# fchchen/omni-recall-rag

Measured on AMD Instinct MI355X. Metric: queries/sec at top-k=10 over N x 3072-d chunks; score delta vs C# reference in `parity`, higher is better.
Workload: dtype i8 screen + f32*f32->f64 exact re-score; 1 GPU; C3: 10000000 chunks x 3072-d fp32 on one GPU, batch=256 queries per step, top-k=10, full hybrid (cosine+keyword+recency), candidate_limit=corpus; corpus_rows=10000000

## Files before the change

include/omnirecall_hip.h:

```cpp
#ifndef OMNIRECALL_HIP_H
#define OMNIRECALL_HIP_H

#include <stddef.h>
#include <stdint.h>

#ifdef __cplusplus
extern "C" {
#endif

#define ORR_ABI_VERSION 1

typedef enum orr_status {
    ORR_OK      = 0,
    ORR_EINVAL  = -1,
    ORR_ENOMEM  = -2,
    ORR_EDEVICE = -3,
    ORR_ECOMM   = -4,
    ORR_EDIM    = -5,
    ORR_ESTATE  = -6,
    ORR_ELIMIT  = -7
} orr_status;

typedef struct orr_index orr_index;

// ... 233 lines not shown
int orr_index_get_rows(orr_index *idx, int64_t n, const int64_t *row_ids , int32_t dim,
                       float *out_emb , uint8_t *out_found );

int orr_search_shard_in_scope(orr_index *idx, int32_t B, int32_t dim, const float *q,
                              const uint8_t *terms_utf8, const uint32_t *term_off, const uint32_t *query_term_off,
                              int64_t now_ticks, int32_t kprime, int64_t candidate_limit, int32_t topk, int32_t pass,
                              const orr_scope *scope, int64_t scope_before, orr_candidate *out);

int orr_search_shard_in_scopes(orr_index *idx, int32_t B, int32_t dim, const float *q,
                               const uint8_t *terms_utf8, const uint32_t *term_off, const uint32_t *query_term_off,
                               int64_t now_ticks, int32_t kprime, int64_t candidate_limit, int32_t topk, int32_t pass,
                               int32_t n_scopes, const orr_scope *const *scopes, const int32_t *query_scope ,
                               const int64_t *scope_before , orr_candidate *out);

int orr_index_set_option(orr_index *idx, const char *name, int64_t value);

int orr_index_screen_dots(orr_index *idx, int32_t B, int32_t dim, const float *q, float *out);

int orr_index_screen_i8_dots(orr_index *idx, int32_t B, int32_t dim, const float *q, int32_t form, int32_t nt_rows,
                             int32_t *out_dots, int8_t *out_iq, int8_t *out_ie);

int orr_index_screen_i8_consts(orr_index *idx, int32_t B, int32_t dim, const float *q, float *out_scale, float *out_rel_err,
                               float *out_rel_hat, float *out_rowf, float *out_s1, double *out_err2, double *out_err2_level1,
                               int8_t *out_iq2);

int orr_index_screen_i8_stream_dots(orr_index *idx, int32_t B, int32_t dim, const float *q, int32_t unit16, int32_t *out_dots);

int orr_index_pass_dots(orr_index *idx, int32_t kernel, int32_t B, int32_t dim, const float *q, float *out);

typedef struct orr_screen_capture {
    int32_t B;
    int32_t kth;
    uint32_t cap;
    int32_t screen;
    int32_t tile_form;
    int32_t scope;
    int32_t floor_form;
    int32_t reserved;
    int64_t n;
    int64_t prefix_rows;
    double eps3;
    double eps1;
} orr_screen_capture;
int orr_index_capture_screen(orr_index *idx, int32_t enabled);
int orr_index_captured_screen(orr_index *idx, orr_screen_capture *info, int32_t B, uint32_t cap, uint64_t *out_floor_key, double *out_L,
                              uint32_t *out_cnt, uint64_t *out_key, uint32_t *out_pos);

int orr_index_pair_dots(orr_index *idx, int32_t n_lists, const uint32_t *list_off ,
                        const int64_t *positions , int32_t stride ,
                        double *out );

int orr_index_keyword_bitmaps(orr_index *idx, int32_t n_terms, const uint8_t *terms_utf8, const uint32_t *term_off, int32_t form,
                              int32_t mid, int64_t out_words_per_term, uint32_t *out_bitmaps, uint8_t *out_alias, int64_t *out_info);

int orr_index_set_profiling(orr_index *idx, int32_t enabled);
int orr_index_kernel_stats(orr_index *idx, orr_kernel_stat *out, int32_t cap);

int orr_index_search_stats(orr_index *idx, orr_search_stats *out, int32_t reset);

typedef struct orr_cluster orr_cluster;
int        orr_cluster_create(const int32_t *devices, int32_t n_shards, int32_t dim, int64_t capacity_rows_per_shard,
                              orr_cluster **out);
void       orr_cluster_destroy(orr_cluster *c);
int32_t    orr_cluster_shards(const orr_cluster *c);
orr_index *orr_cluster_shard(orr_cluster *c, int32_t i);
int        orr_cluster_seal(orr_cluster *c);
int64_t    orr_cluster_rows(const orr_cluster *c);
int        orr_cluster_search_batch(orr_cluster *c, int32_t B, int32_t dim, const float *q_host,
                                    const uint8_t *terms_utf8, const uint32_t *term_off,
                                    const uint32_t *query_term_off, int64_t now_ticks, int32_t topk,
                                    int64_t candidate_limit, int64_t *out_rows, double *out_scores,
                                    int32_t *out_counts);
int        orr_cluster_search_batch_scoped(orr_cluster *c, int32_t B, int32_t dim, const float *q_host,
                                           const uint8_t *terms_utf8, const uint32_t *term_off,
                                           const uint32_t *query_term_off, int64_t now_ticks, int32_t topk,
                                           int64_t candidate_limit, int64_t n_scope_ids, const int64_t *scope_ids,
                                           const uint64_t *scope_off, int64_t *out_rows, double *out_scores,
                                           int32_t *out_counts);
int        orr_cluster_search_batch_masked(orr_cluster *c, int32_t B, int32_t dim, const float *q_host,
                                           const uint8_t *terms_utf8, const uint32_t *term_off,
                                           const uint32_t *query_term_off, int64_t now_ticks, int32_t topk,
                                           int64_t candidate_limit, int64_t n_scope_ids, const int64_t *scope_ids,
                                           int64_t *out_rows, double *out_scores, int32_t *out_counts);
int        orr_cluster_search_stats(orr_cluster *c, orr_search_stats *out, int32_t reset);
int        orr_cluster_set_option(orr_cluster *c, const char *name, int64_t value);
int        orr_cluster_compact(orr_cluster *c, int64_t *out_removed);

int        orr_cluster_insert_rows(orr_cluster *c, int32_t shard, int64_t n, int32_t dim, const float *emb,
                                   const int64_t *created_ticks, const uint8_t *content_lower,
                                   const uint64_t *content_off, const int64_t *row_ids, int64_t *out_inserted);

typedef struct orr_cluster_scope orr_cluster_scope;
int     orr_cluster_scope_create(orr_cluster *c, int64_t n_ids, const int64_t *ids , orr_cluster_scope **out);
int     orr_cluster_scope_create_ticks(orr_cluster *c, int64_t ticks_from, int64_t ticks_to, orr_cluster_scope **out);
int     orr_cluster_scope_create_terms(orr_cluster *c, int32_t n_terms, const uint8_t *terms_utf8 , const uint32_t *term_off ,
                                       int32_t mode, orr_cluster_scope **out);
int     orr_cluster_scope_create_near(orr_cluster *c, int32_t n_probes, int32_t dim, const float *probes ,
                                      double min_cosine, int32_t mode, orr_cluster_scope **out);
int     orr_cluster_scope_add_ids(orr_cluster_scope *s, int64_t n_ids, const int64_t *ids , int64_t *out_added);
int     orr_cluster_scope_combine(orr_cluster_scope *dst, int32_t op, const orr_cluster_scope *src);
int64_t orr_cluster_scope_rows(const orr_cluster_scope *s);
int     orr_cluster_scope_row_ids(orr_cluster_scope *s, int64_t cap, int64_t *out_ids , int64_t *out_n);
const orr_scope *orr_cluster_scope_shard(const orr_cluster_scope *s, int32_t i);
void    orr_cluster_scope_destroy(orr_cluster_scope *s);

int orr_cluster_search_batch_in_scope(orr_cluster *c, int32_t B, int32_t dim, const float *q_host,
// ... 59 lines not shown
```

omni-recall-rag_amd/_native.py:

```python
from __future__ import annotations

import ctypes as C
import os

_PKG = os.path.dirname(os.path.abspath(__file__))
HIP_LIB_PATH = os.environ.get("ORR_HIP_LIB") or os.path.join(_PKG, "libomnirecall_hip.so")
HOST_LIB_PATH = os.path.join(_PKG, "libomnirecall_host.so")


class OrrError(RuntimeError):
    def __init__(self, code: int, message: str):
        super().__init__(f"libomnirecall_hip status {code}: {message}")
        self.code = code


ORR_OK, ORR_EINVAL, ORR_ENOMEM, ORR_EDEVICE, ORR_ECOMM, ORR_EDIM, ORR_ESTATE = 0, -1, -2, -3, -4, -5, -6
ORR_ELIMIT = -7
ORR_CAND_TRAILER, ORR_CAND_DOT_EXACT, ORR_CAND_DEAD = 1, 2, 16
ORR_SCOPE_AND, ORR_SCOPE_OR, ORR_SCOPE_ANDNOT = 0, 1, 2
ORR_TERMS_ALL, ORR_TERMS_ANY = 0, 1
ORR_NEAR_ALL, ORR_NEAR_ANY = 0, 1
ORR_KEY_NONE = -(1 << 63)


# ... 122 lines not shown
hip.orr_keys_centroid_index.argtypes = [_vp, _vp, C.POINTER(_vp), _vp, _vp]
hip.orr_index_get_rows.restype = C.c_int
hip.orr_index_get_rows.argtypes = [_vp, _i64, _vp, _i32, _vp, _vp]
hip.orr_search_shard_in_scope.restype = C.c_int
hip.orr_search_shard_in_scope.argtypes = [_vp, _i32, _i32, _vp, _vp, _vp, _vp, _i64, _i32, _i64, _i32, _i32, _vp, _i64, _vp]
hip.orr_search_shard_in_scopes.restype = C.c_int
hip.orr_search_shard_in_scopes.argtypes = [_vp, _i32, _i32, _vp, _vp, _vp, _vp, _i64, _i32, _i64, _i32, _i32, _i32, _vp, _vp, _vp, _vp]
hip.orr_search_shard_ex.restype = C.c_int
hip.orr_search_shard_ex.argtypes = [_vp, _i32, _i32, _vp, _vp, _vp, _vp, _i64, _i32, _i64, _i32, _i32, _vp]
hip.orr_merge_candidates_ex.restype = C.c_int
hip.orr_merge_candidates_ex.argtypes = [_i32, _i32, _i32, _vp, _i32, _i32, _vp, _vp, _i64, _i32, _vp, _vp, _vp, _vp, _vp]
hip.orr_merge_candidates.restype = C.c_int
hip.orr_merge_candidates.argtypes = [_i32, _i32, _i32, _vp, _i32, _i32, _vp, _vp, _i64, _i32, _vp, _vp, _vp, _vp]
hip.orr_index_save.restype = C.c_int
hip.orr_index_save.argtypes = [_vp, C.c_char_p]
hip.orr_index_load.restype = C.c_int
hip.orr_index_load.argtypes = [C.POINTER(OrrConfig), C.c_char_p, C.POINTER(_vp)]
hip.orr_index_set_option.restype = C.c_int
hip.orr_index_set_option.argtypes = [_vp, C.c_char_p, _i64]
hip.orr_index_delete_rows.restype = C.c_int
hip.orr_index_delete_rows.argtypes = [_vp, _i64, _vp, _vp]
hip.orr_index_update_rows.restype = C.c_int
hip.orr_index_update_rows.argtypes = [_vp, _i64, _vp, _i32, _vp, _vp]
hip.orr_index_insert_rows.restype = C.c_int
hip.orr_index_insert_rows.argtypes = [_vp, _i64, _i32, _vp, _vp, _vp, _vp, _vp, _vp]
hip.orr_cluster_insert_rows.restype = C.c_int
hip.orr_cluster_insert_rows.argtypes = [_vp, _i32, _i64, _i32, _vp, _vp, _vp, _vp, _vp, _vp]
hip.orr_index_compact.restype = C.c_int
hip.orr_index_compact.argtypes = [_vp, _vp]
hip.orr_cluster_compact.restype = C.c_int
hip.orr_cluster_compact.argtypes = [_vp, _vp]
hip.orr_index_live_rows.restype = _i64
hip.orr_index_live_rows.argtypes = [_vp]
hip.orr_index_view.restype = C.c_int
hip.orr_index_view.argtypes = [_vp, C.POINTER(_vp)]
hip.orr_index_screen_dots.restype = C.c_int
hip.orr_index_screen_dots.argtypes = [_vp, _i32, _i32, _vp, _vp]
hip.orr_index_screen_i8_dots.restype = C.c_int
hip.orr_index_screen_i8_dots.argtypes = [_vp, _i32, _i32, _vp, _i32, _i32, _vp, _vp, _vp]
hip.orr_index_screen_i8_consts.restype = C.c_int
hip.orr_index_screen_i8_consts.argtypes = [_vp, _i32, _i32, _vp, _vp, _vp, _vp, _vp, _vp, _vp, _vp, _vp]
hip.orr_index_screen_i8_stream_dots.restype = C.c_int
hip.orr_index_screen_i8_stream_dots.argtypes = [_vp, _i32, _i32, _vp, _i32, _vp]
hip.orr_index_pass_dots.restype = C.c_int
hip.orr_index_pass_dots.argtypes = [_vp, _i32, _i32, _i32, _vp, _vp]
hip.orr_index_capture_screen.restype = C.c_int
hip.orr_index_capture_screen.argtypes = [_vp, _i32]
hip.orr_index_captured_screen.restype = C.c_int
hip.orr_index_captured_screen.argtypes = [_vp, C.POINTER(OrrScreenCapture), _i32, C.c_uint32, _vp, _vp, _vp, _vp, _vp]
hip.orr_index_pair_dots.restype = C.c_int
hip.orr_index_pair_dots.argtypes = [_vp, _i32, _vp, _vp, _i32, _vp]
hip.orr_index_keyword_bitmaps.restype = C.c_int
hip.orr_index_keyword_bitmaps.argtypes = [_vp, _i32, _vp, _vp, _i32, _i32, _i64, _vp, _vp, _vp]
hip.orr_index_set_profiling.restype = C.c_int
hip.orr_index_set_profiling.argtypes = [_vp, _i32]
hip.orr_index_kernel_stats.restype = C.c_int
hip.orr_index_kernel_stats.argtypes = [_vp, _vp, _i32]
hip.orr_index_search_stats.restype = C.c_int
hip.orr_index_search_stats.argtypes = [_vp, C.POINTER(OrrSearchStats), _i32]
hip.orr_cluster_create.restype = C.c_int
hip.orr_cluster_create.argtypes = [_vp, _i32, _i32, _i64, C.POINTER(_vp)]
hip.orr_cluster_destroy.restype = None
hip.orr_cluster_destroy.argtypes = [_vp]
hip.orr_cluster_shards.restype = _i32
hip.orr_cluster_shards.argtypes = [_vp]
hip.orr_cluster_shard.restype = _vp
hip.orr_cluster_shard.argtypes = [_vp, _i32]
hip.orr_cluster_seal.restype = C.c_int
hip.orr_cluster_seal.argtypes = [_vp]
hip.orr_cluster_rows.restype = _i64
hip.orr_cluster_rows.argtypes = [_vp]
hip.orr_cluster_search_batch.restype = C.c_int
hip.orr_cluster_search_batch.argtypes = [_vp, _i32, _i32, _vp, _vp, _vp, _vp, _i64, _i32, _i64, _vp, _vp, _vp]
hip.orr_cluster_search_batch_scoped.restype = C.c_int
hip.orr_cluster_search_batch_scoped.argtypes = [_vp, _i32, _i32, _vp, _vp, _vp, _vp, _i64, _i32, _i64, _i64, _vp, _vp, _vp, _vp, _vp]
hip.orr_cluster_search_batch_masked.restype = C.c_int
hip.orr_cluster_search_batch_masked.argtypes = [_vp, _i32, _i32, _vp, _vp, _vp, _vp, _i64, _i32, _i64, _i64, _vp, _vp, _vp, _vp]
hip.orr_cluster_set_option.restype = C.c_int
hip.orr_cluster_set_option.argtypes = [_vp, C.c_char_p, _i64]
hip.orr_cluster_search_stats.restype = C.c_int
hip.orr_cluster_search_stats.argtypes = [_vp, C.POINTER(OrrSearchStats), _i32]
hip.orr_cluster_scope_create.restype = C.c_int
hip.orr_cluster_scope_create.argtypes = [_vp, _i64, _vp, C.POINTER(_vp)]
hip.orr_cluster_scope_create_ticks.restype = C.c_int
hip.orr_cluster_scope_create_ticks.argtypes = [_vp, _i64, _i64, C.POINTER(_vp)]
hip.orr_cluster_scope_create_terms.restype = C.c_int
hip.orr_cluster_scope_create_terms.argtypes = [_vp, _i32, _vp, _vp, _i32, C.POINTER(_vp)]
hip.orr_cluster_scope_create_near.restype = C.c_int
hip.orr_cluster_scope_create_near.argtypes = [_vp, _i32, _i32, _vp, C.c_double, _i32, C.POINTER(_vp)]
hip.orr_cluster_scope_add_ids.restype = C.c_int
hip.orr_cluster_scope_add_ids.argtypes = [_vp, _i64, _vp, _vp]
hip.orr_cluster_scope_combine.restype = C.c_int
hip.orr_cluster_scope_combine.argtypes = [_vp, _i32, _vp]
hip.orr_cluster_scope_rows.restype = _i64
hip.orr_cluster_scope_rows.argtypes = [_vp]
hip.orr_cluster_scope_row_ids.restype = C.c_int
hip.orr_cluster_scope_row_ids.argtypes = [_vp, _i64, _vp, _vp]
hip.orr_cluster_scope_shard.restype = _vp
hip.orr_cluster_scope_shard.argtypes = [_vp, _i32]
hip.orr_cluster_scope_destroy.restype = None
hip.orr_cluster_scope_destroy.argtypes = [_vp]
hip.orr_cluster_search_batch_in_scope.restype = C.c_int
hip.orr_cluster_search_batch_in_scope.argtypes = [_vp, _i32, _i32, _vp, _vp, _vp, _vp, _i64, _i32, _i64, _vp, _vp, _vp, _vp]
hip.orr_cluster_search_batch_in_scopes.restype = C.c_int
hip.orr_cluster_search_batch_in_scopes.argtypes = [_vp, _i32, _i32, _vp, _vp, _vp, _vp, _i64, _i32, _i64, _i32, _vp, _vp, _vp, _vp, _vp]
hip.orr_cluster_search_range_cosine.restype = C.c_int
# ... 55 lines not shown
host.orrh_store_import_cosmos_json.restype = C.c_int
host.orrh_store_import_cosmos_json.argtypes = [_vp, C.c_char_p, _i64, _vp, _vp]
host.orrh_store_export_cosmos_json.restype = C.c_int
host.orrh_store_export_cosmos_json.argtypes = [_vp, C.POINTER(_vp), C.POINTER(_i64)]
host.orrh_store_chunk_count.restype = _i64
host.orrh_store_chunk_count.argtypes = [_vp]
host.orrh_service_create.restype = _vp
host.orrh_service_create.argtypes = [_vp, _i32, _i64]
host.orrh_service_stats.restype = None
host.orrh_service_stats.argtypes = [_vp, _vp, _vp, _vp]
host.orrh_service_tombstoned_rows.restype = _i64
host.orrh_service_tombstoned_rows.argtypes = [_vp]
host.orrh_service_compactions.restype = _i64
host.orrh_service_compactions.argtypes = [_vp]
host.orrh_service_delta_merges.restype = _i64
host.orrh_service_delta_merges.argtypes = [_vp]
host.orrh_service_updated_rows.restype = _i64
host.orrh_service_updated_rows.argtypes = [_vp]
host.orrh_service_inserted_rows.restype = _i64
host.orrh_service_inserted_rows.argtypes = [_vp]
host.orrh_service_set_option.restype = C.c_int
host.orrh_service_set_option.argtypes = [_vp, C.c_char_p, _i64]
host.orrh_service_destroy.restype = None
host.orrh_service_destroy.argtypes = [_vp]
host.orrh_service_search_json.restype = C.c_int
host.orrh_service_search_json.argtypes = [_vp, C.c_char_p, _vp, _i32, _i32, _i64, C.POINTER(_vp), C.POINTER(_i64)]
host.orrh_service_search_documents_json.restype = C.c_int
host.orrh_service_search_documents_json.argtypes = [_vp, C.c_char_p, _vp, _i32, _i32, _i64, C.POINTER(C.c_char_p), _i32, C.POINTER(_vp), C.POINTER(_i64)]
host.orrh_free.restype = None
host.orrh_free.argtypes = [_vp]
host.orrh_batcher_create.restype = _vp
host.orrh_batcher_create.argtypes = [_vp, _i32, _i32]
host.orrh_batcher_destroy.restype = None
host.orrh_batcher_destroy.argtypes = [_vp]
host.orrh_batcher_search.restype = C.c_int
host.orrh_batcher_search.argtypes = [_vp, _i32, _vp, _vp, _vp, _i32, _i64, _i32, _i64, _vp, _vp, _vp]
host.orrh_batcher_search_at.restype = C.c_int
host.orrh_batcher_search_at.argtypes = [_vp, _i32, _vp, _vp, _vp, _i32, _i64, _i32, _i64, _vp, _vp, _vp, _vp]
host.orrh_batcher_stats.restype = None
host.orrh_batcher_stats.argtypes = [_vp, _vp, _vp, _vp]
host.orrh_batcher_create.restype = _vp
host.orrh_batcher_create.argtypes = [_vp, _i32, _i32]
host.orrh_batcher_destroy.restype = None
host.orrh_batcher_destroy.argtypes = [_vp]
host.orrh_batcher_search.restype = C.c_int
host.orrh_batcher_search.argtypes = [_vp, _i32, _vp, _vp, _vp, _i32, _i64, _i32, _i64, _vp, _vp, _vp]
host.orrh_batcher_stats.restype = None
host.orrh_batcher_stats.argtypes = [_vp, _vp, _vp, _vp]

EXPORTED_HIP_SYMBOLS = [
    "orr_abi_version", "orr_device_count", "orr_last_error", "orr_index_create", "orr_index_destroy",
    "orr_index_append", "orr_index_seal", "orr_index_rows", "orr_index_dim", "orr_search_batch",
    "orr_search_shard", "orr_search_shard_ex", "orr_search_batch_scoped", "orr_search_batch_masked", "orr_search_batch_masked_groups", "orr_search_shard_scoped", "orr_search_shard_masked", "orr_index_scope_count", "orr_merge_candidates", "orr_merge_candidates_ex", "orr_index_set_profiling", "orr_index_kernel_stats",
    "orr_index_save", "orr_index_load", "orr_index_set_row_base", "orr_index_set_option", "orr_index_screen_dots", "orr_index_screen_i8_dots", "orr_index_screen_i8_consts", "orr_index_screen_i8_stream_dots", "orr_index_pass_dots", "orr_index_capture_screen", "orr_index_captured_screen", "orr_index_keyword_bitmaps", "orr_index_view",
    "orr_index_delete_rows", "orr_index_update_rows", "orr_index_insert_rows", "orr_cluster_insert_rows", "orr_index_live_rows", "orr_index_compact", "orr_cluster_compact", "orr_index_search_stats",
    "orr_cluster_create", "orr_cluster_destroy", "orr_cluster_shards", "orr_cluster_shard", "orr_cluster_seal", "orr_cluster_rows",
    "orr_cluster_search_batch", "orr_cluster_search_batch_scoped", "orr_cluster_search_batch_masked", "orr_cluster_search_stats", "orr_cluster_set_option",
    "orr_scope_create", "orr_scope_create_ticks", "orr_scope_create_terms", "orr_scope_create_near", "orr_scope_add_ids", "orr_scope_combine", "orr_scope_rows", "orr_scope_row_ids", "orr_scope_destroy",
    "orr_search_batch_in_scope", "orr_search_batch_in_scopes", "orr_search_shard_in_scope", "orr_search_shard_in_scopes", "orr_search_range_cosine", "orr_search_range_cosine_bulk",
    "orr_search_batch_diverse", "orr_index_pair_dots",
    "orr_keys_create", "orr_keys_set", "orr_keys_get", "orr_keys_rows", "orr_keys_destroy", "orr_scope_create_keys", "orr_search_batch_per_key",
    "orr_keys_groups", "orr_keys_centroids", "orr_scope_centroid",
    "orr_keys_centroid_index", "orr_index_get_rows",
    "orr_cluster_scope_create", "orr_cluster_scope_create_ticks", "orr_cluster_scope_create_terms", "orr_cluster_scope_create_near", "orr_cluster_scope_add_ids", "orr_cluster_scope_combine",
    "orr_cluster_scope_rows", "orr_cluster_scope_row_ids", "orr_cluster_scope_shard", "orr_cluster_scope_destroy", "orr_cluster_search_batch_in_scope",
    "orr_cluster_search_batch_in_scopes", "orr_cluster_search_range_cosine", "orr_cluster_search_range_cosine_bulk",
    "orr_cluster_search_batch_diverse", "orr_cluster_pair_dots",
    "orr_cluster_keys_create", "orr_cluster_keys_set", "orr_cluster_keys_get", "orr_cluster_keys_rows", "orr_cluster_keys_shard", "orr_cluster_keys_destroy",
    "orr_cluster_scope_create_keys", "orr_cluster_search_batch_per_key",
    "orr_cluster_keys_groups", "orr_cluster_keys_centroids", "orr_cluster_scope_centroid",
]
EXPORTED_HOST_SYMBOLS = ["orrh_is_blank", "orrh_lower_invariant", "orrh_query_terms", "orrh_build_snippet",
                         "orrh_round4", "orrh_has_sufficient_evidence", "orrh_format_score_f4", "orrh_last_error", "orrh_store_create", "orrh_store_destroy",
                         "orrh_store_upsert_document", "orrh_store_upsert_chunks", "orrh_store_delete_document",
                         "orrh_store_chunk_count", "orrh_store_import_cosmos_json", "orrh_store_export_cosmos_json", "orrh_service_create", "orrh_service_destroy",
                         "orrh_service_search_json", "orrh_service_search_documents_json", "orrh_service_stats", "orrh_service_tombstoned_rows", "orrh_service_compactions", "orrh_service_delta_merges", "orrh_service_updated_rows", "orrh_service_inserted_rows", "orrh_service_set_option", "orrh_free", "orrh_batcher_create", "orrh_batcher_destroy",
                         "orrh_batcher_search", "orrh_batcher_search_at", "orrh_batcher_stats"]


def check(status: int) -> None:
    if status != ORR_OK:
        raise OrrError(status, (hip.orr_last_error() or b"").decode("utf-8", "replace"))
```

omni-recall-rag_amd/csrc/orr_api.hip:

```cpp
#include <hip/hip_runtime.h>

#include <algorithm>
#include <cmath>
#include <cstdarg>
#include <cstdio>
#include <chrono>
#include <pthread.h>
#include <dlfcn.h>
#include <atomic>
#include <condition_variable>
#include <functional>
#include <cstring>
#include <limits>
#include <mutex>
#include <shared_mutex>
#include <deque>
#include <new>
#include <numeric>
#include <string>
#include <string_view>
#include <thread>
#include <unordered_map>
#include <vector>

// ... 5382 lines not shown
            HIP_TRY(orr::launch_scope_terms_bases(kws.view.term_word_off, n_distinct, words, lane->ws_scope_terms.as<int64_t>(), h_base, k));
        }
        {
            Timed t(lane, "scope_terms_combine", 4.0 * (double)words * ((double)n_distinct + 1.0), k);
            HIP_TRY(orr::launch_scope_terms_combine(kws.view.bitmaps, lane->ws_scope_terms.as<int64_t>(), n_distinct, mode, words, lane->n_rows, sc->bm, k));
        }
        HIP_TRY(hipEventRecord(lane->ev_kw_done, k));
        HIP_TRY(hipStreamSynchronize(k));
        const int verdict = check_hit_list(lane, kws, "orr_scope_create_terms");
        if (verdict != ORR_OK && verdict != kRetryPass) return verdict;
        ORR_TRY(clean_keyword_side(lane, kws, (uint32_t)n_terms));
        if (verdict == kRetryPass) {
            if (attempt + 1 >= keyword::kMaxRuns) return hit_list_kept_overflowing("orr_scope_create_terms");
            continue;
        }
        if (h_base) {
            int64_t aliased = 0;
            for (int32_t t = 0; t < n_distinct; ++t) aliased += h_base[t] != (int64_t)t * words;
            lane->stats[(size_t)stat_slot(lane, "scope_terms_aliased")].algo_bytes += 4.0 * (double)words * (double)aliased;
        }
        break;
    }
    HIP_TRY(hipStreamWaitEvent(lane->stream, lane->ev_kw_done, 0));
    Timed t(lane, "scope_clear_positions", 12.0 * (double)own->dead.size());
    HIP_TRY(orr::launch_scope_clear_positions(sc->bm, sc->words, own->d_dead.as<int64_t>(), (int64_t)own->dead.size(), lane->stream));
    return ORR_OK;
}

static int scope_fill_terms(orr_index *lane, orr_scope *sc, int32_t n_terms, const uint8_t *terms_utf8, const uint32_t *term_off, int32_t mode)
{
    const int r = scope_fill_terms_run(lane, sc, n_terms, terms_utf8, term_off, mode);
    if (r != ORR_OK) (void)hipStreamSynchronize(lane->stream_kw);
    return r;
}

int orr_scope_create_terms(orr_index *idx, int32_t n_terms, const uint8_t *terms_utf8, const uint32_t *term_off, int32_t mode, orr_scope **out)
{
    if (!out) return fail(ORR_EINVAL, "orr_scope_create_terms: out is NULL");
    if (!scope_terms::terms_valid(n_terms)) return fail(ORR_EINVAL, "orr_scope_create_terms: n_terms must be in 0 .. %d", scope_terms::kMaxTerms);
    if (n_terms > 0 && (!terms_utf8 || !term_off)) return fail(ORR_EINVAL, "orr_scope_create_terms: terms_utf8 or term_off is NULL with %d terms", n_terms);
    if (!scope_terms::mode_valid(mode)) return fail(ORR_EINVAL, "orr_scope_create_terms: mode must be ORR_TERMS_ALL (0) or ORR_TERMS_ANY (1)");
    const int32_t bad = scope_terms::first_bad_term(term_off, n_terms);
    if (bad >= 0 && term_off[bad + 1] == term_off[bad]) return fail(ORR_EINVAL, "orr_scope_create_terms: term %d is empty", bad);
    if (bad >= 0) return fail(ORR_EINVAL, "orr_scope_create_terms: term_off is not monotone at term %d", bad);
    if (!idx) return fail(ORR_EINVAL, "orr_scope_create_terms: null index");
    return make_scope(idx, "orr_scope_create_terms", out, [&](orr_index *lane, orr_scope *sc) -> int {
        return scope_fill_terms(lane, sc, n_terms, terms_utf8, term_off, mode);
    });
}

constexpr int32_t kKwDiagMaxTerms = 4096;
constexpr uint64_t kKwDiagMaxBytes = (uint64_t)1 << 30;

static int keyword_bitmaps_run(orr_index *lane, int32_t n_terms, const uint8_t *terms_utf8, const uint32_t *term_off, int64_t words,
                               uint32_t *out_bitmaps, uint8_t *out_alias, int64_t *out_info)
{
    const uint32_t query_term_off[2] = {0u, (uint32_t)n_terms};
    BatchArgs a{1, 0, nullptr, terms_utf8, term_off, query_term_off, 0, 0};
    const std::vector<uint32_t> qoff(query_term_off, query_term_off + 2);
    hipStream_t k = lane->stream_kw;
    std::vector<int64_t> h_off((size_t)n_terms);
    std::vector<uint8_t> h_alias((size_t)n_terms, 0);
    for (int attempt = 0;; ++attempt) {
        KwSide kws;
        ORR_TRY(launch_keyword_side(lane, a, qoff, kws));
        if (kws.view.words_per_term != words || kws.bm_bytes != sizeof(uint32_t) * (size_t)n_terms * (size_t)words)
            return fail(ORR_ESTATE, "orr_index_keyword_bitmaps: the keyword side made %zu bytes of bitmaps of %lld words for %d terms",
                        kws.bm_bytes, (long long)kws.view.words_per_term, n_terms);
        const bool has_store = kws.view.term_word_off != nullptr && kws.alias != nullptr;
        if (has_store) {
            HIP_TRY(hipMemcpyAsync(h_off.data(), kws.view.term_word_off, sizeof(int64_t) * (size_t)n_terms, hipMemcpyDeviceToHost, k));
            HIP_TRY(hipMemcpyAsync(h_alias.data(), kws.alias, (size_t)n_terms, hipMemcpyDeviceToHost, k));
        }
        HIP_TRY(hipStreamSynchronize(k));
        const uint32_t hits = (uint32_t)(*lane->pin_kwcnt.as<unsigned long long>() >> 32);
        const int verdict = check_hit_list(lane, kws, "orr_index_keyword_bitmaps");
        if (verdict != ORR_OK && verdict != kRetryPass) return verdict;
        if (verdict == ORR_OK) {
            HIP_TRY(hipMemcpyAsync(out_bitmaps, kws.view.bitmaps, kws.bm_bytes, hipMemcpyDeviceToHost, k));
            for (int32_t t = 0; has_store && t < n_terms; ++t)
                if (h_off[(size_t)t] != (int64_t)t * words)
                    HIP_TRY(hipMemcpyAsync(out_bitmaps + (size_t)t * (size_t)words, kws.view.bitmaps + h_off[(size_t)t], sizeof(uint32_t) * (size_t)words,
                                           hipMemcpyDeviceToHost, k));
            HIP_TRY(hipStreamSynchronize(k));
        }
        ORR_TRY(clean_keyword_side(lane, kws, (uint32_t)n_terms));
        if (verdict == kRetryPass) {
            if (attempt + 1 >= keyword::kMaxRuns) return hit_list_kept_overflowing("orr_index_keyword_bitmaps");
            continue;
        }
        if (out_alias) memcpy(out_alias, h_alias.data(), (size_t)n_terms);
        out_info[1] = (int64_t)hits;
        out_info[2] = attempt + 1;
        out_info[3] = lane->kw_form_ran;
        break;
    }
    return ORR_OK;
}

int orr_index_keyword_bitmaps(orr_index *idx, int32_t n_terms, const uint8_t *terms_utf8, const uint32_t *term_off, int32_t form, int32_t mid,
                              int64_t out_words_per_term, uint32_t *out_bitmaps, uint8_t *out_alias, int64_t *out_info)
{
    static const char *fn = "orr_index_keyword_bitmaps";
    if (!out_bitmaps || !out_info) return fail(ORR_EINVAL, "%s: out_bitmaps or out_info is NULL", fn);
    if (n_terms < 1 || n_terms > kKwDiagMaxTerms) return fail(ORR_EINVAL, "%s: n_terms must be in 1 .. %d", fn, kKwDiagMaxTerms);
    if (!terms_utf8 || !term_off) return fail(ORR_EINVAL, "%s: terms_utf8 or term_off is NULL", fn);
    if (form < -1 || form > 1) return fail(ORR_EINVAL, "%s: form must be -1 (as a search chooses), 0 (all-pairs) or 1 (lookup)", fn);
    if (mid < -1 || mid > 0) return fail(ORR_EINVAL, "%s: mid must be -1 (default) or 0 (tokens of 17..32 bytes through the wave scan)", fn);
    const int32_t bad = scope_terms::first_bad_term(term_off, n_terms);
    if (bad >= 0 && term_off[bad + 1] == term_off[bad]) return fail(ORR_EINVAL, "%s: term %d is empty", fn, bad);
    if (bad >= 0) return fail(ORR_EINVAL, "%s: term_off is not monotone at term %d", fn, bad);
    {
        std::vector<std::string_view> sorted((size_t)n_terms);
        for (int32_t t = 0; t < n_terms; ++t)
            sorted[(size_t)t] = std::string_view(reinterpret_cast<const char *>(terms_utf8) + term_off[t], term_off[t + 1] - term_off[t]);
        std::sort(sorted.begin(), sorted.end());
        if (std::adjacent_find(sorted.begin(), sorted.end()) != sorted.end()) return fail(ORR_EINVAL, "%s: the terms are not distinct", fn);
    }
    if (!idx) return fail(ORR_EINVAL, "%s: null index", fn);
    Lane ln = acquire_lane(idx);
    orr_index *lane = ln.lane;
    std::lock_guard<std::mutex> lock(lane->mu);
    if (!lane->sealed) return fail(ORR_ESTATE, "%s: the index is not sealed", fn);
    const int64_t words = keyword::words_per_term(lane->n_rows);
    if (out_words_per_term != words) return fail(ORR_EINVAL, "%s: a term bitmap of this shard has %lld words, not %lld", fn, (long long)words, (long long)out_words_per_term);
    if ((uint64_t)n_terms * (uint64_t)words * sizeof(uint32_t) > kKwDiagMaxBytes)
        return fail(ORR_EINVAL, "%s: %d bitmaps of %lld words are more than the %llu bytes a call returns", fn, n_terms, (long long)words, (unsigned long long)kKwDiagMaxBytes);
    out_info[0] = words; out_info[1] = 0; out_info[2] = 0; out_info[3] = -1;
    if (out_alias) memset(out_alias, 0, (size_t)n_terms);
    if (lane->n_rows <= 0) return ORR_OK;
    ORR_TRY(bind_device(lane));
    struct Overrides {
        orr_index *l;
        ~Overrides() { l->kw_force_form = l->kw_force_mid = -1; }
    } overrides{lane};
    lane->kw_force_form = form;
    lane->kw_force_mid = mid;
    const int r = keyword_bitmaps_run(lane, n_terms, terms_utf8, term_off, words, out_bitmaps, out_alias, out_info);
    if (r != ORR_OK) (void)hipStreamSynchronize(lane->stream_kw);
    collect_events(lane);
    return r;
}

static int scope_add_ids_held(orr_index *lane, orr_scope *s, int64_t n_ids, const int64_t *ids, int64_t *out_added)
{
    ORR_TRY(bind_device(lane));
    const int64_t before = s->live.load();
    int r = scope_or_ids(lane, s, n_ids, ids);
    if (r == ORR_OK) r = refresh_scope(lane, s);
    if (r != ORR_OK) { (void)hipStreamSynchronize(lane->stream); return r; }
    if (out_added) *out_added = s->live.load() - before;
    return ORR_OK;
}

static int scope_combine_held(orr_index *lane, orr_scope *dst, int32_t op, const orr_scope *src)
{
    if (dst->words != src->words) return fail(ORR_ESTATE, "orr_scope_combine: the scopes cover different row counts");
    ORR_TRY(bind_device(lane));
    {
        Timed t(lane, "scope_combine", 12.0 * (double)dst->words);
        HIP_TRY(orr::launch_scope_combine(dst->bm, src->bm, dst->words, op, lane->stream));
    }
    const int r = refresh_scope(lane, dst);
    if (r != ORR_OK) (void)hipStreamSynchronize(lane->stream);
    return r;
}

static int scope_row_ids_held(orr_index *lane, const orr_scope *s, int64_t live, int64_t *out_ids)
{
    ORR_TRY(bind_device(lane));
    hipStream_t st = lane->stream;
    const uint32_t ecap = scope::slice_cap((uint32_t)live);
    DevBuf entries, d_ids;
    auto body = [&]() -> int {
        ORR_TRY(entries.reserve(sizeof(orr::SelEntry) * (size_t)ecap));
        ORR_TRY(d_ids.reserve(sizeof(int64_t) * (size_t)live));
        ORR_TRY(lane->pin_scope.reserve(16));
        ORR_TRY(lane->ws_scope_meta.reserve(8));
        ORR_TRY(lane->ws_scope_sel.reserve(sizeof(uint32_t)));
        *lane->pin_scope.as<int64_t>() = live;
        HIP_TRY(hipMemcpyAsync(lane->ws_scope_meta.p, lane->pin_scope.p, 8, hipMemcpyHostToDevice, st));
        HIP_TRY(hipMemsetAsync(lane->ws_scope_sel.p, 0, sizeof(uint32_t), st));
        HIP_TRY(orr::launch_scope_compact(s->bm, s->words, 1, s->chunks, lane->ws_scope_sel.as<uint32_t>(), 1, lane->ws_scope_meta.as<int64_t>(),
                                          entries.as<orr::SelEntry>(), ecap, st));
        HIP_TRY(orr::launch_scope_entry_ids(entries.as<orr::SelEntry>(), live, lane->d_row_ids, lane->n_rows, d_ids.as<int64_t>(), st));
        HIP_TRY(hipMemcpyAsync(out_ids, d_ids.p, sizeof(int64_t) * (size_t)live, hipMemcpyDeviceToHost, st));
        HIP_TRY(hipStreamSynchronize(st));
        return ORR_OK;
    };
    const int r = body();
    if (r != ORR_OK) (void)hipStreamSynchronize(st);
// ... 4277 lines not shown
```

omni-recall-rag_amd/csrc/orr_gemm.hip:

```cpp
#include "orr_kernels.h"
#include "orr_device.h"
#include "orr_epilogue.h"

#include <algorithm>
#include <cstdio>
#include <vector>
#include <cstdlib>

namespace orr {

typedef float f32x4v __attribute__((ext_vector_type(4)));

constexpr int kGemmBK = 64;


constexpr int kBfLd = 72;

__device__ __forceinline__ void split_write(__bf16 *hi_img, __bf16 *lo_img, int r, int c4, const float4 &v)
{
    const __bf16 h0 = (__bf16)v.x, h1 = (__bf16)v.y, h2 = (__bf16)v.z, h3 = (__bf16)v.w;
    bf16x4 h, l;
    h[0] = h0; h[1] = h1; h[2] = h2; h[3] = h3;
    l[0] = (__bf16)(v.x - (float)h0);
    l[1] = (__bf16)(v.y - (float)h1);
// ... 216 lines not shown
            }
        }
#pragma unroll
        for (int k = 0; k < 4; ++k) {
#pragma unroll
            for (int p = 0; p < kCountPlanes; ++p) {
                uint32_t x = c[k][p];
#pragma unroll
                for (int s = 4; s >= 0; --s) {
                    const int jj = 1 << s;
                    const uint32_t low = s == 4 ? 0x0000FFFFu : s == 3 ? 0x00FF00FFu : s == 2 ? 0x0F0F0F0Fu : s == 1 ? 0x33333333u : 0x55555555u;
                    const uint32_t y = (uint32_t)__shfl_xor((int)x, jj, 64);
                    x = (q & jj) ? (((y & ~low) >> jj) | (x & ~low)) : ((x & low) | ((y & low) << jj));
                }
                c[k][p] = x;
            }
            const int64_t row = (Q * 4 + k) * 32 + q;
            if (BITS == 2) {
                if (row < n_rows) {
#pragma unroll
                    for (int kk = 0; kk < 2; ++kk) {
                        uint32_t wv = 0u;
#pragma unroll
                        for (int p = 0; p < 2; ++p) {
                            uint32_t x = (c[k][p] >> (16 * kk)) & 0xFFFFu;
                            x = (x | (x << 8)) & 0x00FF00FFu;
                            x = (x | (x << 4)) & 0x0F0F0F0Fu;
                            x = (x | (x << 2)) & 0x33333333u;
                            x = (x | (x << 1)) & 0x55555555u;
                            wv |= x << p;
                        }
                        planes[((int64_t)kk * n_qg + g) * plane_stride + row] = wv;
                    }
                }
            } else if (row < n_rows) {
#pragma unroll
                for (int kk = 0; kk < 4; ++kk) {
                    uint32_t wv = 0u;
#pragma unroll
                    for (int p = 0; p < kCountPlanes; ++p) {
                        uint32_t x = (c[k][p] >> (8 * kk)) & 0xFFu;
                        x = (x | (x << 12)) & 0x000F000Fu;
                        x = (x | (x << 6)) & 0x03030303u;
                        x = (x | (x << 3)) & 0x11111111u;
                        wv |= x << p;
                    }
                    planes[((int64_t)kk * n_qg + g) * plane_stride + row] = wv;
                }
            }
        }
    }
}

hipError_t launch_query_count_planes(KwView kw, int32_t B, int64_t n_rows, int64_t plane_stride, uint32_t *planes, hipStream_t s,
                                     int64_t row_first, int64_t row_end, int32_t bits)
{
    if (B <= 0 || !kw.bitmaps || n_rows <= 0) return hipSuccess;
    if (kw.words_per_term % 4 != 0 || row_first % 256 != 0) return hipErrorInvalidValue;
    const int64_t n_oct = (kw.words_per_term / 4 + 1) / 2;
    const int64_t oct_first = row_first / 256;
    const int64_t oct_end = row_end < 0 ? n_oct : std::min<int64_t>(n_oct, (row_end + 255) / 256);
    if (oct_end <= oct_first) return hipSuccess;
    int64_t bx = (oct_end - oct_first + 3) / 4;
    if (bx > 2048) bx = 2048;
    if (bits == 2)
        hipLaunchKernelGGL(query_count_planes_kernel<2>, dim3((unsigned)bx, (unsigned)((B + 31) / 32)), dim3(256), 0, s, kw, B, n_rows,
                           plane_stride, planes, oct_first, oct_end);
    else
        hipLaunchKernelGGL(query_count_planes_kernel<4>, dim3((unsigned)bx, (unsigned)((B + 31) / 32)), dim3(256), 0, s, kw, B, n_rows,
                           plane_stride, planes, oct_first, oct_end);
    return hipGetLastError();
}

__device__ __forceinline__ float4 fused_query_const_of(const QueryConst &c, unsigned long long tau_b, const float *i8_qs1, const double *i8_qerr2, int b)
{
    float4 o;
    o.x = c.use_cos ? (float)(c.inv_sqrt_na * 0.7) : 0.f;
    if (tau_b <= 1ull) {
        o.y = -__builtin_huge_valf();
    } else {
        const double floor_score = key_score(tau_b);
        const double margin = 1e-5 * (1.0 + fabs(floor_score));
        o.y = __double2float_rd(floor_score - margin);
    }
    o.z = c.n_terms > 0 ? __double2float_ru(0.2 / (double)(c.n_terms > 15 ? 15 : c.n_terms)) : 0.f;
    o.w = 0.f;
    if (i8_qs1) {
        o.x *= i8_qs1[b];
        o.w = c.use_cos ? __double2float_ru(0.7 * 1.000001 * sqrt(i8_qerr2[b]) * c.inv_sqrt_na) : 0.f;
    }
    return o;
}

__global__ __launch_bounds__(256) void fused_query_consts_kernel(const QueryConst *__restrict__ qc,
                                                                 const unsigned long long *__restrict__ tau, int32_t B,
                                                                 float4 *__restrict__ qf, const float *__restrict__ i8_qs1,
                                                                 const double *__restrict__ i8_qerr2, float4 *__restrict__ qf16,
                                                                 uint32_t *__restrict__ zero_a, int32_t n_a, uint32_t *__restrict__ zero_b,
                                                                 int32_t n_b)
{
    __shared__ float red[4];
    for (int i = threadIdx.x; i < n_a; i += 256) zero_a[i] = 0u;
    for (int i = threadIdx.x; i < n_b; i += 256) zero_b[i] = 0u;
    float wmax = 0.f;
    for (int b = threadIdx.x; b < B; b += 256) {
        const float4 o = fused_query_const_of(qc[b], tau[b], i8_qs1, i8_qerr2, b);
        qf[b] = o;
        const bool fin = o.x >= 0.f && o.x <= 1.0f && o.w >= 0.f && o.w <= 1e30f && o.z >= 0.f && o.z <= 1.f && o.y == o.y;
        if (fin) wmax = fmaxf(wmax, o.w);
    }
    if (!qf16) return;
#pragma unroll
    for (int d = 32; d > 0; d >>= 1) wmax = fmaxf(wmax, __shfl_xor(wmax, d, 64));
    if ((threadIdx.x & 63) == 0) red[threadIdx.x >> 6] = wmax;
    __syncthreads();
// ... 1113 lines not shown
```

Measured before the change: 31620 queries/s.

## Add transpose-based two-bit keyword count kernel and count-words diagnostic API

Adds a new kernel for the two-bit query count planes. It loads term bitmap words per lane, adds up to three terms with bit-sliced half adders, then uses a 32x32 bit transpose and a swizzled shared-memory stage to write per-row count words with vectorized stores. The old bit-spreading kernel is kept for the four-bit case and for unaligned outputs. A new orr_index_count_words entry point exposes the count planes to the host for checking. The new kernel covers the whole word range in one grid instead of capping the grid at 2048 blocks, and it relies on 16-byte alignment of the planes pointer.

```diff
diff --git a/include/omnirecall_hip.h b/include/omnirecall_hip.h
--- a/include/omnirecall_hip.h
+++ b/include/omnirecall_hip.h
@@ -309,6 +309,10 @@
 
 int orr_index_keyword_bitmaps(orr_index *idx, int32_t n_terms, const uint8_t *terms_utf8, const uint32_t *term_off, int32_t form,
                               int32_t mid, int64_t out_words_per_term, uint32_t *out_bitmaps, uint8_t *out_alias, int64_t *out_info);
+
+int orr_index_count_words(orr_index *idx, int32_t B, const uint8_t *terms_utf8, const uint32_t *term_off,
+                          const uint32_t *query_term_off , int32_t bits, int64_t row_first, int64_t row_end,
+                          int64_t plane_stride, uint32_t *words);
 
 int orr_index_set_profiling(orr_index *idx, int32_t enabled);
 int orr_index_kernel_stats(orr_index *idx, orr_kernel_stat *out, int32_t cap);
diff --git a/omni-recall-rag_amd/_native.py b/omni-recall-rag_amd/_native.py
--- a/omni-recall-rag_amd/_native.py
+++ b/omni-recall-rag_amd/_native.py
@@ -198,6 +198,8 @@
 hip.orr_index_pair_dots.argtypes = [_vp, _i32, _vp, _vp, _i32, _vp]
 hip.orr_index_keyword_bitmaps.restype = C.c_int
 hip.orr_index_keyword_bitmaps.argtypes = [_vp, _i32, _vp, _vp, _i32, _i32, _i64, _vp, _vp, _vp]
+hip.orr_index_count_words.restype = C.c_int
+hip.orr_index_count_words.argtypes = [_vp, _i32, _vp, _vp, _vp, _i32, _i64, _i64, _i64, _vp]
 hip.orr_index_set_profiling.restype = C.c_int
 hip.orr_index_set_profiling.argtypes = [_vp, _i32]
 hip.orr_index_kernel_stats.restype = C.c_int
@@ -359,7 +361,7 @@
     "orr_abi_version", "orr_device_count", "orr_last_error", "orr_index_create", "orr_index_destroy",
     "orr_index_append", "orr_index_seal", "orr_index_rows", "orr_index_dim", "orr_search_batch",
     "orr_search_shard", "orr_search_shard_ex", "orr_search_batch_scoped", "orr_search_batch_masked", "orr_search_batch_masked_groups", "orr_search_shard_scoped", "orr_search_shard_masked", "orr_index_scope_count", "orr_merge_candidates", "orr_merge_candidates_ex", "orr_index_set_profiling", "orr_index_kernel_stats",
-    "orr_index_save", "orr_index_load", "orr_index_set_row_base", "orr_index_set_option", "orr_index_screen_dots", "orr_index_screen_i8_dots", "orr_index_screen_i8_consts", "orr_index_screen_i8_stream_dots", "orr_index_pass_dots", "orr_index_capture_screen", "orr_index_captured_screen", "orr_index_keyword_bitmaps", "orr_index_view",
+    "orr_index_save", "orr_index_load", "orr_index_set_row_base", "orr_index_set_option", "orr_index_screen_dots", "orr_index_screen_i8_dots", "orr_index_screen_i8_consts", "orr_index_screen_i8_stream_dots", "orr_index_pass_dots", "orr_index_capture_screen", "orr_index_captured_screen", "orr_index_keyword_bitmaps", "orr_index_count_words", "orr_index_view",
     "orr_index_delete_rows", "orr_index_update_rows", "orr_index_insert_rows", "orr_cluster_insert_rows", "orr_index_live_rows", "orr_index_compact", "orr_cluster_compact", "orr_index_search_stats",
     "orr_cluster_create", "orr_cluster_destroy", "orr_cluster_shards", "orr_cluster_shard", "orr_cluster_seal", "orr_cluster_rows",
     "orr_cluster_search_batch", "orr_cluster_search_batch_scoped", "orr_cluster_search_batch_masked", "orr_cluster_search_stats", "orr_cluster_set_option",
diff --git a/omni-recall-rag_amd/csrc/orr_api.hip b/omni-recall-rag_amd/csrc/orr_api.hip
--- a/omni-recall-rag_amd/csrc/orr_api.hip
+++ b/omni-recall-rag_amd/csrc/orr_api.hip
@@ -5458,31 +5458,52 @@
 constexpr int32_t kKwDiagMaxTerms = 4096;
 constexpr uint64_t kKwDiagMaxBytes = (uint64_t)1 << 30;
 
+struct CountWordsDiag {
+    int32_t B, bits;
+    const uint32_t *query_term_off;
+    int64_t row_first, row_end, plane_stride;
+    uint32_t *words;
+};
+
 static int keyword_bitmaps_run(orr_index *lane, int32_t n_terms, const uint8_t *terms_utf8, const uint32_t *term_off, int64_t words,
-                               uint32_t *out_bitmaps, uint8_t *out_alias, int64_t *out_info)
-{
-    const uint32_t query_term_off[2] = {0u, (uint32_t)n_terms};
-    BatchArgs a{1, 0, nullptr, terms_utf8, term_off, query_term_off, 0, 0};
-    const std::vector<uint32_t> qoff(query_term_off, query_term_off + 2);
+                               uint32_t *out_bitmaps, uint8_t *out_alias, int64_t *out_info, const CountWordsDiag *cw = nullptr)
+{
+    const char *fn = cw ? "orr_index_count_words" : "orr_index_keyword_bitmaps";
+    const uint32_t one_query[2] = {0u, (uint32_t)n_terms};
+    const uint32_t *query_term_off = cw ? cw->query_term_off : one_query;
+    const int32_t B = cw ? cw->B : 1;
+    BatchArgs a{B, 0, nullptr, terms_utf8, term_off, query_term_off, 0, 0};
+    const std::vector<uint32_t> qoff(query_term_off, query_term_off + B + 1);
     hipStream_t k = lane->stream_kw;
+    const size_t cw_bytes = cw ? sizeof(uint32_t) * (size_t)cw->bits * (size_t)((B + 31) / 32) * (size_t)cw->plane_stride : 0;
+    if (cw) ORR_TRY(lane->ws_fany.reserve(cw_bytes));
     std::vector<int64_t> h_off((size_t)n_terms);
     std::vector<uint8_t> h_alias((size_t)n_terms, 0);
     for (int attempt = 0;; ++attempt) {
         KwSide kws;
         ORR_TRY(launch_keyword_side(lane, a, qoff, kws));
-        if (kws.view.words_per_term != words || kws.bm_bytes != sizeof(uint32_t) * (size_t)n_terms * (size_t)words)
+        if (!cw && (kws.view.words_per_term != words || kws.bm_bytes != sizeof(uint32_t) * (size_t)n_terms * (size_t)words))
             return fail(ORR_ESTATE, "orr_index_keyword_bitmaps: the keyword side made %zu bytes of bitmaps of %lld words for %d terms",
                         kws.bm_bytes, (long long)kws.view.words_per_term, n_terms);
-        const bool has_store = kws.view.term_word_off != nullptr && kws.alias != nullptr;
+        if (cw) {
+            HIP_TRY(hipMemcpyAsync(lane->ws_fany.p, cw->words, cw_bytes, hipMemcpyHostToDevice, k));
+            Timed t(lane, "count_planes", (cw->bits == 2 ? 8.0 : 16.0) * (double)((B + 31) / 32) * (double)lane->n_rows, k);
+            HIP_TRY(orr::launch_query_count_planes(kws.view, B, lane->n_rows, cw->plane_stride, lane->ws_fany.as<uint32_t>(), k, cw->row_first,
+                                                   cw->row_end, cw->bits));
+        }
+        const bool has_store = !cw && kws.view.term_word_off != nullptr && kws.alias != nullptr;
         if (has_store) {
             HIP_TRY(hipMemcpyAsync(h_off.data(), kws.view.term_word_off, sizeof(int64_t) * (size_t)n_terms, hipMemcpyDeviceToHost, k));
             HIP_TRY(hipMemcpyAsync(h_alias.data(), kws.alias, (size_t)n_terms, hipMemcpyDeviceToHost, k));
         }
         HIP_TRY(hipStreamSynchronize(k));
         const uint32_t hits = (uint32_t)(*lane->pin_kwcnt.as<unsigned long long>() >> 32);
-        const int verdict = check_hit_list(lane, kws, "orr_index_keyword_bitmaps");
+        const int verdict = check_hit_list(lane, kws, fn);
         if (verdict != ORR_OK && verdict != kRetryPass) return verdict;
-        if (verdict == ORR_OK) {
+        if (verdict == ORR_OK && cw) {
+            HIP_TRY(hipMemcpyAsync(cw->words, lane->ws_fany.p, cw_bytes, hipMemcpyDeviceToHost, k));
+            HIP_TRY(hipStreamSynchronize(k));
+        } else if (verdict == ORR_OK) {
             HIP_TRY(hipMemcpyAsync(out_bitmaps, kws.view.bitmaps, kws.bm_bytes, hipMemcpyDeviceToHost, k));
             for (int32_t t = 0; has_store && t < n_terms; ++t)
                 if (h_off[(size_t)t] != (int64_t)t * words)
@@ -5492,13 +5513,15 @@
         }
         ORR_TRY(clean_keyword_side(lane, kws, (uint32_t)n_terms));
         if (verdict == kRetryPass) {
-            if (attempt + 1 >= keyword::kMaxRuns) return hit_list_kept_overflowing("orr_index_keyword_bitmaps");
+            if (attempt + 1 >= keyword::kMaxRuns) return hit_list_kept_overflowing(fn);
             continue;
         }
         if (out_alias) memcpy(out_alias, h_alias.data(), (size_t)n_terms);
-        out_info[1] = (int64_t)hits;
-        out_info[2] = attempt + 1;
-        out_info[3] = lane->kw_form_ran;
+        if (out_info) {
+            out_info[1] = (int64_t)hits;
+            out_info[2] = attempt + 1;
+            out_info[3] = lane->kw_form_ran;
+        }
         break;
     }
     return ORR_OK;
@@ -5543,6 +5566,40 @@
     lane->kw_force_form = form;
     lane->kw_force_mid = mid;
     const int r = keyword_bitmaps_run(lane, n_terms, terms_utf8, term_off, words, out_bitmaps, out_alias, out_info);
+    if (r != ORR_OK) (void)hipStreamSynchronize(lane->stream_kw);
+    collect_events(lane);
+    return r;
+}
+
+int orr_index_count_words(orr_index *idx, int32_t B, const uint8_t *terms_utf8, const uint32_t *term_off, const uint32_t *query_term_off,
+                          int32_t bits, int64_t row_first, int64_t row_end, int64_t plane_stride, uint32_t *words)
+{
+    static const char *fn = "orr_index_count_words";
+    if (!words || !query_term_off) return fail(ORR_EINVAL, "%s: words or query_term_off is NULL", fn);
+    if (B < 1 || B > 1024) return fail(ORR_EINVAL, "%s: B must be in 1 .. 1024", fn);
+    if (bits != 2 && bits != 4) return fail(ORR_EINVAL, "%s: bits must be 2 or 4", fn);
+    if (row_first < 0 || row_first % 256 != 0) return fail(ORR_EINVAL, "%s: row_first must be a multiple of 256", fn);
+    uint32_t max_terms = 0;
+    for (int32_t b = 0; b < B; ++b) {
+        if (query_term_off[b + 1] < query_term_off[b]) return fail(ORR_EINVAL, "%s: query_term_off is not monotone at query %d", fn, b);
+        max_terms = std::max(max_terms, query_term_off[b + 1] - query_term_off[b]);
+    }
+    if (query_term_off[0] != 0) return fail(ORR_EINVAL, "%s: query_term_off must start at 0", fn);
+    const int32_t n_terms = (int32_t)query_term_off[B];
+    if (n_terms > 0 && (!terms_utf8 || !term_off)) return fail(ORR_EINVAL, "%s: terms_utf8 or term_off is NULL", fn);
+    if (bits == 2 && max_terms > 3) return fail(ORR_EINVAL, "%s: two-bit count words hold at most three terms a query", fn);
+    const int32_t bad = n_terms > 0 ? scope_terms::first_bad_term(term_off, n_terms) : -1;
+    if (bad >= 0) return fail(ORR_EINVAL, "%s: term %d is empty or term_off is not monotone there", fn, bad);
+    if (!idx) return fail(ORR_EINVAL, "%s: null index", fn);
+    Lane ln = acquire_lane(idx);
+    orr_index *lane = ln.lane;
+    std::lock_guard<std::mutex> lock(lane->mu);
+    if (!lane->sealed) return fail(ORR_ESTATE, "%s: the index is not sealed", fn);
+    if (plane_stride < lane->n_rows || plane_stride < 1) return fail(ORR_EINVAL, "%s: plane_stride must be at least the shard's %lld rows", fn, (long long)lane->n_rows);
+    if (lane->n_rows <= 0 || n_terms == 0) return ORR_OK;
+    ORR_TRY(bind_device(lane));
+    const CountWordsDiag cw{B, bits, query_term_off, row_first, row_end, plane_stride, words};
+    const int r = keyword_bitmaps_run(lane, n_terms, terms_utf8, term_off, 0, nullptr, nullptr, nullptr, &cw);
     if (r != ORR_OK) (void)hipStreamSynchronize(lane->stream_kw);
     collect_events(lane);
     return r;
diff --git a/omni-recall-rag_amd/csrc/orr_gemm.hip b/omni-recall-rag_amd/csrc/orr_gemm.hip
--- a/omni-recall-rag_amd/csrc/orr_gemm.hip
+++ b/omni-recall-rag_amd/csrc/orr_gemm.hip
@@ -292,6 +292,135 @@
     }
 }
 
+namespace count_words2 {
+
+constexpr int kBlockQueries = 8, kSlots = 3;
+
+template <int S>
+__host__ __device__ constexpr void transpose32_step(uint32_t (&m)[32])
+{
+    constexpr uint32_t low = S == 16 ? 0x0000FFFFu : S == 8 ? 0x00FF00FFu : S == 4 ? 0x0F0F0F0Fu : S == 2 ? 0x33333333u : 0x55555555u;
+#pragma unroll
+    for (int j = 0; j < 16; ++j) {
+        const int i = ((j & ~(S - 1)) << 1) | (j & (S - 1));
+        const uint32_t a = m[i], b = m[i | S];
+        m[i] = (a & low) | ((b & low) << S);
+        m[i | S] = ((a >> S) & low) | (b & ~low);
+    }
+}
+__host__ __device__ constexpr void transpose32(uint32_t (&m)[32])
+{
+    transpose32_step<16>(m); transpose32_step<8>(m); transpose32_step<4>(m); transpose32_step<2>(m); transpose32_step<1>(m);
+}
+
+constexpr bool transpose32_exact()
+{
+    uint32_t m[32] = {}, x = 0x9E3779B9u;
+    for (int i = 0; i < 32; ++i) { x = x * 1664525u + 1013904223u; m[i] = x ^ (x >> 15); }
+    uint32_t t[32] = {};
+    for (int i = 0; i < 32; ++i) t[i] = m[i];
+    transpose32(t);
+    for (int r = 0; r < 32; ++r)
+        for (int i = 0; i < 32; ++i)
+            if (((t[r] >> i) & 1u) != ((m[i] >> r) & 1u)) return false;
+    return true;
+}
+static_assert(transpose32_exact(), "count words: bit i of m[r] must become bit r of m[i]");
+
+}
+
+__global__ __launch_bounds__(256) void query_count_words2_kernel(KwView kw, int32_t B, int64_t n_rows, int64_t plane_stride,
+                                                                uint32_t *__restrict__ planes, int64_t word_first, int64_t word_end)
+{
+    using namespace count_words2;
+    __shared__ uint4 slots[32 * kSlots];
+    __shared__ uint4 stage[4 * 64 * 8];
+    const int g = blockIdx.y;
+    const int32_t n_qg = gridDim.y;
+    const int lane = threadIdx.x & 63;
+    if (threadIdx.x < 32 * kSlots) {
+        const int q = (int)threadIdx.x / kSlots, j = (int)threadIdx.x % kSlots, b = g * 32 + q;
+        uint32_t t0 = 0, t1 = 0;
+        if (b < B) { t0 = kw.q_term_off[b]; t1 = kw.q_term_off[b + 1]; }
+        const bool has_term = t0 + (uint32_t)j < t1;
+        const uint32_t term = kw.q_term_idx[has_term ? t0 + j : t0 < t1 ? t0 : 0u];
+        const uint64_t at = reinterpret_cast<uint64_t>(kw.bitmaps + kw_term_base(kw, term));
+        slots[threadIdx.x] = make_uint4((uint32_t)at, (uint32_t)(at >> 32), has_term ? ~0u : 0u, 0u);
+    }
+    __syncthreads();
+    const int64_t word0 = word_first + ((int64_t)blockIdx.x * 4 + __builtin_amdgcn_readfirstlane((int)(threadIdx.x >> 6))) * 64;
+    if (word0 >= word_end) return;
+    const int64_t word = word0 + lane;
+    const bool has_bits = word < kw.words_per_term;
+    const uint64_t load_off = (uint64_t)(has_bits ? word : kw.words_per_term - 1) * 4u;
+
+    auto issue = [&](uint32_t (&w)[kBlockQueries][kSlots], int q0) {
+#pragma unroll
+        for (int q = 0; q < kBlockQueries; ++q)
+#pragma unroll
+            for (int j = 0; j < kSlots; ++j) {
+                const uint4 sl = slots[(q0 + q) * kSlots + j];
+                w[q][j] = *reinterpret_cast<gptr<uint32_t>>((((uint64_t)sl.y << 32) | sl.x) + load_off);
+            }
+    };
+
+    uint32_t cur[kBlockQueries][kSlots], nxt[kBlockQueries][kSlots];
+    issue(cur, 0);
+#pragma unroll
+    for (int kk = 0; kk < 2; ++kk) {
+        uint32_t m[32];
+#pragma unroll
+        for (int half = 0; half < 2; ++half) {
+            const int q0 = 16 * kk + kBlockQueries * half;
+            if (q0 + kBlockQueries < 32) issue(nxt, q0 + kBlockQueries);
+            __builtin_amdgcn_sched_barrier(0);
+#pragma unroll
+            for (int q = 0; q < kBlockQueries; ++q) {
+                uint32_t c0 = 0u, c1 = 0u;
+#pragma unroll
+                for (int j = 0; j < kSlots; ++j) {
+                    const uint32_t w = cur[q][j] & slots[(q0 + q) * kSlots + j].z;
+                    c1 ^= c0 & w;
+                    c0 ^= w;
+                }
+                m[2 * (kBlockQueries * half + q)] = c0;
+                m[2 * (kBlockQueries * half + q) + 1] = c1;
+            }
+            if (q0 + kBlockQueries < 32) {
+#pragma unroll
+                for (int q = 0; q < kBlockQueries; ++q)
+#pragma unroll
+                    for (int j = 0; j < kSlots; ++j) cur[q][j] = nxt[q][j];
+            }
+        }
+        transpose32(m);
+        if (!has_bits) {
+#pragma unroll
+            for (int r = 0; r < 32; ++r) m[r] = 0u;
+        }
+        {
+            uint4 *mine = stage + (threadIdx.x >> 6) * (64 * 8);
+#pragma unroll
+            for (int c = 0; c < 8; ++c) mine[lane * 8 + (c ^ ((lane >> 1) & 7))] = make_uint4(m[4 * c], m[4 * c + 1], m[4 * c + 2], m[4 * c + 3]);
+            uint32_t *out = planes + ((int64_t)kk * n_qg + g) * plane_stride;
+            const int64_t row_end = word_end * 32 < n_rows ? word_end * 32 : n_rows;
+#pragma unroll
+            for (int i = 0; i < 8; ++i) {
+                const int line = 8 * i + (lane >> 3);
+                const uint4 v = mine[line * 8 + ((lane & 7) ^ ((line >> 1) & 7))];
+                const int64_t row = (word0 + line) * 32 + 4 * (lane & 7);
+                if (row + 4 <= row_end) {
+                    *reinterpret_cast<uint4 *>(out + row) = v;
+                } else {
+                    if (row < row_end) out[row] = v.x;
+                    if (row + 1 < row_end) out[row + 1] = v.y;
+                    if (row + 2 < row_end) out[row + 2] = v.z;
+                }
+            }
+        }
+    }
+}
+
 hipError_t launch_query_count_planes(KwView kw, int32_t B, int64_t n_rows, int64_t plane_stride, uint32_t *planes, hipStream_t s,
                                      int64_t row_first, int64_t row_end, int32_t bits)
 {
@@ -301,6 +430,13 @@
     const int64_t oct_first = row_first / 256;
     const int64_t oct_end = row_end < 0 ? n_oct : std::min<int64_t>(n_oct, (row_end + 255) / 256);
     if (oct_end <= oct_first) return hipSuccess;
+    if (bits == 2 && plane_stride % 4 == 0 && (reinterpret_cast<uintptr_t>(planes) & 15u) == 0) {
+        const int64_t word_first = oct_first * 8, word_end = oct_end * 8;
+        const int64_t waves = (word_end - word_first + 63) / 64;
+        hipLaunchKernelGGL(query_count_words2_kernel, dim3((unsigned)((waves + 3) / 4), (unsigned)((B + 31) / 32)), dim3(256), 0, s, kw, B,
+                           n_rows, plane_stride, planes, word_first, word_end);
+        return hipGetLastError();
+    }
     int64_t bx = (oct_end - oct_first + 3) / 4;
     if (bx > 2048) bx = 2048;
     if (bits == 2)
```

After: 32100 queries/s, median of 6. +1.5%, better.
